# GloryyrolG/MHEntropy

Hardware: AMD Instinct MI355X
Metric: hypotheses/sec (BxK) fwd+loss, 256x256 (higher is better)
Workload: dtype bf16; 1 GPU; c2: MHEnt.get_loss forward+loss, resnet50 encoder (train-mode BN), 12-coupling RealNVP h=512, MANO joints, B=256/GPU, K=64, 256x256; images_per_gpu=256, hypotheses_per_image=64, global_batch=256, launch=hip-graph replay, base_noise=drawn on the device inside the step (Philox4x32-10, mhe_randn_f32), timing=one window of 452 steps, bracketed by barrier + synchronize, ranks=1, rccl_ranks=0

## Files before the change

mhentropy_amd/csrc/conv.hip:

```cpp
#include "conv_shared.h"
#include <cstdlib>

namespace mhe { namespace conv {

template <typename T, int BM, int BN, int WM, int WN, bool FAST, int MODE, bool DG = false>
__global__ __launch_bounds__(64 * WM * WN, WM * WN == 4 ? 2 : 1) void conv_kernel(const Params p) {
    constexpr int NTH = 64 * WM * WN;
    constexpr int CE = El<T>::CE, BKE = 8 * CE;
    constexpr int RSTEP = NTH / 8;
    constexpr int NJ_A = BM / RSTEP, NJ_B = BN / RSTEP;
    constexpr int MTW = BM / WM / 16, NTW = BN / WN / 16;
    __shared__ uint4 lds[2][(BM + BN) * 8];
    constexpr bool AFFM = MODE == 1 || MODE == 2;
    __shared__ __attribute__((aligned(16))) float aff[2][AFFM ? MAXC : 4];

    const int tid = threadIdx.x, wave = tid >> 6, lane = tid & 63;
    const int q = lane >> 4, l15 = lane & 15;
    const int wr = wave / WN, wc = wave % WN;
    int mtile, ntile;
    tile_of_block(mtile, ntile);
    const int m0 = mtile * BM, n0 = ntile * BN;
    const int s = tid & 7, rbase = tid >> 3;
    const T *xg = reinterpret_cast<const T *>(p.x);
    const T *wg = reinterpret_cast<const T *>(p.w);
// ... 657 lines not shown
extern "C" int mhe_conv1x1_cat_bias_nhwc(const mhe_conv_desc *d, const void *x, const void *xcat, int cin2, const void *w, void *y, const void *residual,
                                         const float *bias, void *stream) {
    MHE_REQUIRE(d && xcat && d->dtype == MHE_BF16 && d->KH == 1 && d->KW == 1 && d->stride == 1 && d->pad == 0 && cin2 > 0 && cin2 % 64 == 0 && d->Cin % 64 == 0,
                "mhe_conv1x1_cat_bias_nhwc: a bf16 1x1 stride-1 launch on two operand tensors with Cin and cin2 multiples of 64");
    MHE_REQUIRE(d->tile == 0 || d->tile == 1 || d->tile == 2, "mhe_conv1x1_cat_bias_nhwc: 128-row register-staged tiles only (tile 0, 1 or 2)");
    ConvRequest r;
    r.x = x; r.w = w; r.y = y; r.out_shift = bias; r.residual = residual; r.xcat = xcat; r.cin2 = cin2;
    return conv_entry(d, r, stream);
}

extern "C" int mhe_conv1x1_residual_in_masked_nhwc(const mhe_conv_desc *d, const void *x, const void *x2, const void *w, void *y,
                                                   const float *in_scale, const float *in_shift, const float *x2_scale,
                                                   const float *x2_shift, void *a_out, const void *residual, const void *mask,
                                                   const void *bn_y0, const float *bn_mean_invstd0, mhe_stat_t *bn_stats0, void *stream) {
    MHE_REQUIRE(d && x2 && in_scale && in_shift && mask, "mhe_conv1x1_residual_in_masked_nhwc: x2, in_scale, in_shift and mask are required");
    MHE_REQUIRE(d->KH == 1 && d->KW == 1 && d->stride == 1 && d->pad == 0, "mhe_conv1x1_residual_in_masked_nhwc: 1x1 stride-1 only");
    MHE_REQUIRE((x2_scale == nullptr) == (x2_shift == nullptr), "mhe_conv1x1_residual_in_masked_nhwc: x2_scale/x2_shift must come together");
    ConvRequest r;
    r.x = x; r.w = w; r.y = y; r.in_scale = in_scale; r.in_shift = in_shift; r.x2 = x2; r.x2_scale = x2_scale; r.x2_shift = x2_shift; r.a_out = a_out;
    if (int rc = bn_rev(r.bn, "mhe_conv1x1_residual_in_masked_nhwc", 1, {{bn_y0}, {bn_mean_invstd0}, {bn_stats0}})) return rc;
    MHE_REQUIRE(d->tile == 0 || d->tile == 1 || d->tile == 2 || d->tile == 11,
                "mhe_conv1x1_residual_in_masked_nhwc: 128-row tiles only (tile 0, 1, 2, or 11 = the transfer-wave kernel)");
    r.residual = residual; r.mask = mask;
    return conv_entry(d, r, stream);
}

extern "C" int mhe_conv2d_masked_nhwc(const mhe_conv_desc *d, const void *x, const void *w, void *y, const void *residual,
                                      const void *mask, const void *bn_y0, const float *bn_mean_invstd0, mhe_stat_t *bn_stats0,
                                      const void *bn_y1, const float *bn_mean_invstd1, mhe_stat_t *bn_stats1, void *stream) {
    MHE_REQUIRE(mask, "mhe_conv2d_masked_nhwc: mask is required");
    ConvRequest r;
    if (int rc = bn_rev(r.bn, "mhe_conv2d_masked_nhwc", 2, {{bn_y0, bn_y1}, {bn_mean_invstd0, bn_mean_invstd1}, {bn_stats0, bn_stats1}})) return rc;
    r.x = x; r.w = w; r.y = y; r.residual = residual; r.mask = mask;
    return conv_entry(d, r, stream);
}

extern "C" int mhe_conv2d_masked_bits_nhwc(const mhe_conv_desc *d, const void *x, const void *w, void *y, const void *residual,
                                           const void *mask, const void *mask_bits, const void *bn_y0, const float *bn_mean_invstd0, mhe_stat_t *bn_stats0,
                                           const void *bn_y1, const float *bn_mean_invstd1, mhe_stat_t *bn_stats1, void *stream) {
    MHE_REQUIRE(mask, "mhe_conv2d_masked_bits_nhwc: mask is required (kernels without the bit path read it)");
    ConvRequest r;
    if (int rc = bn_rev(r.bn, "mhe_conv2d_masked_bits_nhwc", 2, {{bn_y0, bn_y1}, {bn_mean_invstd0, bn_mean_invstd1}, {bn_stats0, bn_stats1}})) return rc;
    MHE_REQUIRE(!mask_bits || (d && d->Cout % 8 == 0), "mhe_conv2d_masked_bits_nhwc: Cout must be a multiple of 8");
    r.x = x; r.w = w; r.y = y; r.residual = residual; r.mask = mask; r.mask_bits = mask_bits;
    return conv_entry(d, r, stream);
}

extern "C" int mhe_conv2d_masked_bias_nhwc(const mhe_conv_desc *d, const void *x, const void *xcat, int cin2, const void *w, void *y,
                                           const void *residual, const void *mask, const float *bias, const void *bn_y0,
                                           const float *bn_mean_invstd0, mhe_stat_t *bn_stats0, void *stream) {
    MHE_REQUIRE(mask && bias, "mhe_conv2d_masked_bias_nhwc: mask and bias are required");
    MHE_REQUIRE(!xcat || (d && d->dtype == MHE_BF16 && d->KH == 1 && d->KW == 1 && d->stride == 1 && d->pad == 0 && cin2 > 0 && cin2 % 64 == 0 && d->Cin % 64 == 0),
                "mhe_conv2d_masked_bias_nhwc: a concatenated operand needs a bf16 1x1 stride-1 launch with Cin and cin2 multiples of 64");
    ConvRequest r;
    if (int rc = bn_rev(r.bn, "mhe_conv2d_masked_bias_nhwc", 1, {{bn_y0}, {bn_mean_invstd0}, {bn_stats0}})) return rc;
    MHE_REQUIRE(d && (d->tile == 0 || d->tile == 1 || d->tile == 2), "mhe_conv2d_masked_bias_nhwc: 128-row register-staged tiles only (tile 0, 1 or 2)");
    r.x = x; r.w = w; r.y = y; r.out_shift = bias; r.residual = residual; r.mask = mask; r.xcat = xcat; r.cin2 = xcat ? cin2 : 0;
    return conv_entry(d, r, stream);
}

extern "C" int mhe_conv3x3s2_dgrad_nhwc(int B, int Ho, int Wo, int Cout, int Cin, int dtype, const void *gy, const void *const *w4,
                                        void *dx, const void *residual, const void *mask, const void *bn_y0,
                                        const float *bn_mean_invstd0, mhe_stat_t *bn_stats0, const void *bn_y1,
                                        const float *bn_mean_invstd1, mhe_stat_t *bn_stats1, int tile, void *stream) {
    MHE_REQUIRE(gy && w4 && dx && w4[0] && w4[1] && w4[2] && w4[3], "mhe_conv3x3s2_dgrad_nhwc: null pointer");
    MHE_REQUIRE((!bn_y0 || (bn_mean_invstd0 && bn_stats0 && mask)) && (!bn_y1 || (bn_y0 && bn_mean_invstd1 && bn_stats1)),
                "mhe_conv3x3s2_dgrad_nhwc: each bn_y needs its mean_invstd and stats (and the gate)");
    ConvRequest r;
    r.x = gy; r.y = dx; r.residual = residual; r.mask = mask;
    if (mask) r.bn = {{bn_y0, bn_y1}, {bn_mean_invstd0, bn_mean_invstd1}, {bn_stats0, bn_stats1}};
    for (int py = 0; py < 2; ++py)
        for (int px = 0; px < 2; ++px) {
            mhe_conv_desc d = {B, Ho, Wo, Cout, Cin, 1 + py, 1 + px, 1, 0, dtype, 0, 0, tile};
            const int sc[2] = {py, px};
            r.w = w4[2 * py + px]; r.scatter = sc;
            if (int rc = conv_entry(&d, r, stream)) return rc;
        }
    return MHE_OK;
}

extern "C" int mhe_conv1x1_stats_nhwc(const mhe_conv_desc *d, const void *x, const void *w, const float *in_scale, const float *in_shift,
                                      mhe_stat_t *stats, void *stream) {
    MHE_REQUIRE(d && x && w && stats, "mhe_conv1x1_stats_nhwc: null pointer");
    MHE_REQUIRE(d->dtype == MHE_BF16 && d->KH == 1 && d->KW == 1 && d->stride == 1 && d->pad == 0 && (d->Cin == 64 || d->Cin == 128 || d->Cin == 256) && d->Cout % 256 == 0,
                "mhe_conv1x1_stats_nhwc: bf16 1x1 stride-1 with 64 / 128 / 256 input channels and a multiple of 256 output channels");
    MHE_REQUIRE((in_scale == nullptr) == (in_shift == nullptr), "mhe_conv1x1_stats_nhwc: in_scale/in_shift must come together");
    conv::Params p{};
    p.x = x; p.w = w; p.y = nullptr; p.in_scale = in_scale; p.in_shift = in_shift; p.stats = stats;
    const long long M = conv::fill_geometry(p, *d);
    MHE_REQUIRE(M > 0 && M < (1ll << 31), "mhe_conv1x1_stats_nhwc: bad pixel count");
    p.relu_in = d->relu_in; p.force = 8; p.stats_only = 1;
    if (d->Cin == 256) {
        p.force = 11;
        MHE_REQUIRE(conv::wide_supports(p), "mhe_conv1x1_stats_nhwc: geometry not taken by the resident-slab kernel (M=%lld Cout=%d)", M, d->Cout);
        return conv::launch_wide(p, (hipStream_t)stream);
    }
    MHE_REQUIRE(conv::stream_supports(p), "mhe_conv1x1_stats_nhwc: geometry not taken by the streaming kernel");
    return conv::launch_stream(p, (hipStream_t)stream);
}

extern "C" int mhe_bottleneck_tail_supported(const mhe_conv_desc *d, int Cb) {
    if (!d || d->dtype != MHE_BF16) return 0;
    static const float dummy = 0.f;
    conv::Params p{};
    p.x = p.x2 = p.w = p.w3 = p.y = p.a_out = (void *)&dummy; p.in_scale = p.in_shift = p.mid_scale = p.mid_shift = &dummy;
    const long long M = conv::fill_geometry(p, *d, true);
    if (M <= 0 || M >= (1ll << 31)) return 0;
    return conv::fuse_supports(p, Cb) ? 1 : 0;
}

static int bottleneck_tail(const char *entry, const mhe_conv_desc *d, int Cb, conv::Params &p, void *stream) {
    MHE_REQUIRE(d && p.x && p.in_scale && p.in_shift && p.w3 && p.mid_scale && p.mid_shift && p.x2 && p.w && p.a_out && p.y, "%s: null pointer", entry);
    MHE_REQUIRE(d->dtype == MHE_BF16, "%s: bf16 storage only", entry);
    MHE_REQUIRE((p.x2_scale == nullptr) == (p.x2_shift == nullptr), "%s: id_scale/id_shift must come together", entry);
    MHE_REQUIRE(!p.a_quarter || (d->B > 0 && d->H > 0 && d->W > 0), "%s: bad geometry", entry);
    p.relu_in = 1; p.force = -1;
    const long long M = conv::fill_geometry(p, *d, true);
    MHE_REQUIRE(M > 0 && (p.a_quarter ? M * d->Cin : M) < (1ll << 31), "%s: bad pixel count", entry);
    MHE_REQUIRE(conv::fuse_supports(p, Cb), "%s: needs Cin = 4 Cb, Cb 64 / 128, Cout 64 / 128, pixels %% 128 == 0 (Cin=%d Cb=%d Cout=%d M=%lld)",
                entry, d->Cin, Cb, d->Cout, M);
    return conv::launch_fuse(p, Cb, (hipStream_t)stream);
}

extern "C" int mhe_bottleneck_tail_nhwc(const mhe_conv_desc *d, int Cb, const void *y2, const float *bn2_scale, const float *bn2_shift,
                                        const void *w3, const float *bn3_scale, const float *bn3_shift, const void *identity,
                                        const float *id_scale, const float *id_shift, const void *w1, void *a_out, void *y1, mhe_stat_t *stats,
                                        void *stream) {
    return mhe_bottleneck_tail_bits_nhwc(d, Cb, y2, bn2_scale, bn2_shift, w3, bn3_scale, bn3_shift, identity, id_scale, id_shift, w1, a_out, nullptr, y1, stats, stream);
}

extern "C" int mhe_bottleneck_tail_bits_nhwc(const mhe_conv_desc *d, int Cb, const void *y2, const float *bn2_scale, const float *bn2_shift,
                                             const void *w3, const float *bn3_scale, const float *bn3_shift, const void *identity,
                                             const float *id_scale, const float *id_shift, const void *w1, void *a_out, void *a_bits, void *y1,
                                             mhe_stat_t *stats, void *stream) {
    conv::Params p{};
    p.x = y2; p.in_scale = bn2_scale; p.in_shift = bn2_shift; p.w3 = w3; p.mid_scale = bn3_scale; p.mid_shift = bn3_shift;
    p.x2 = identity; p.x2_scale = id_scale; p.x2_shift = id_shift; p.w = w1; p.a_out = a_out; p.y = y1; p.stats = stats;
    p.a_bits = (unsigned char *)a_bits;
    return bottleneck_tail("mhe_bottleneck_tail_nhwc", d, Cb, p, stream);
}

extern "C" int mhe_bottleneck_tail_quarter_nhwc(const mhe_conv_desc *d, int Cb, const void *y2, const float *bn2_scale, const float *bn2_shift,
                                                const void *w3, const float *bn3_scale, const float *bn3_shift, const void *identity,
                                                const float *id_scale, const float *id_shift, const void *w1, void *a_quarter, void *y1,
                                                mhe_stat_t *stats, void *stream) {
    conv::Params p{};
    p.x = y2; p.in_scale = bn2_scale; p.in_shift = bn2_shift; p.w3 = w3; p.mid_scale = bn3_scale; p.mid_shift = bn3_shift;
    p.x2 = identity; p.x2_scale = id_scale; p.x2_shift = id_shift; p.w = w1; p.a_out = a_quarter; p.y = y1; p.stats = stats;
    p.a_quarter = 1;
    return bottleneck_tail("mhe_bottleneck_tail_quarter_nhwc", d, Cb, p, stream);
}

extern "C" int mhe_conv_stat_shards(void) { return conv::NSH; }
extern "C" size_t mhe_stat_words(int C) { return C > 0 ? (size_t)2 * conv::NSH * 2 * (size_t)C : 0; }

extern "C" int mhe_conv_tile_mode(const mhe_conv_desc *d, int mode) {
    if (!d || mode < 0 || mode > 3) return -1;
    static const float dummy = 0.f;
    conv::Params p{};
    conv::fill_geometry(p, *d);
    p.force = d->tile - 1;
    if (mode == 1 || mode == 2) p.in_scale = &dummy;
    if (mode == 2) p.x2 = &dummy;
    if (mode == 3) p.residual = &dummy;
    return conv::choose_tile(p, d->Cin % (8 * conv::elem_chunk(d->dtype)) == 0, d->dtype == MHE_BF16);
}

// ... 244 lines not shown
```

mhentropy_amd/csrc/conv_wide.hip:

```cpp
#include "conv_shared.h"

namespace mhe { namespace conv {

namespace {
constexpr int WBM = 128, WBK = 64, WSLAB = 64 * 1024 / 16;
constexpr int WNSET = 8;
typedef unsigned int u32x4 __attribute__((ext_vector_type(4)));
}

template <int NS, int NK, bool BNLOAD>
__global__ __launch_bounds__(512) void conv_wide_kernel(const Params p, int nslab, int tiles_per_wg) {
    using T = u16;
    constexpr int CPR = NS / 8;
    constexpr int TPI = WNSET / NK;
    __shared__ uint4 Wl[WSLAB];
    __shared__ uint4 Al[3][WBM * 8];
    __shared__ uint4 Ol[WBM * CPR];
    __shared__ float aff[BNLOAD ? 2 * 512 : 2];
    const int tid = threadIdx.x, wave = __builtin_amdgcn_readfirstlane(tid >> 6), lane = tid & 63, q = lane >> 4, l15 = lane & 15;
    const bool mult = wave < 4;
    const int t2 = tid & 255, s = t2 & 7, rbase = t2 >> 3;
    constexpr int K = NK * WBK;
    const int xcd = blockIdx.x & 7, a = blockIdx.x >> 3, slab = a % nslab, group = a / nslab, ngroup = 32 / nslab;
    const int n0 = slab * NS;
    const int niter = tiles_per_wg / TPI;
    auto tile_m0 = [&](int j) __attribute__((always_inline)) { return (8 * (group + ngroup * j) + xcd) * WBM; };
    const T *xg = reinterpret_cast<const T *>(p.x), *wg = reinterpret_cast<const T *>(p.w);
    for (int i = tid; i < NS * NK * 8; i += 512) {
        const int c = i & 7, n = (i >> 3) % NS, kt = i / (8 * NS);
        Wl[kt * NS * 8 + swz(n, c)] = *reinterpret_cast<const uint4 *>(wg + (size_t)(n0 + n) * p.Kpad + kt * WBK + c * 8);
    }
    if constexpr (BNLOAD) {
        for (int i = tid; i < K; i += 512) { aff[i] = p.in_scale[i]; aff[512 + i] = p.in_shift[i]; }
    }
    __syncthreads();
    const bool st_on = p.stats != nullptr;
    constexpr int RSTEP = 256 / CPR, NR = WBM / RSTEP;
    float ss1[8], ss2[8];
#pragma unroll
    for (int e = 0; e < 8; ++e) ss1[e] = ss2[e] = 0.f;
    if (mult) {
        constexpr int MT = NS == 128 ? 4 : 2;
        const int px0 = NS == 128 ? (wave >> 1) * 64 : wave * 32, ch0 = NS == 128 ? (wave & 1) * 64 : 0;
        v4f acc[4][MT];
        uint4 fa[2][2][MT], fb[2][2][4];
        auto read_frags = [&](int buf, const uint4 *At, int kt) __attribute__((always_inline)) {
            const uint4 *Wt = Wl + kt * NS * 8;
#pragma unroll
            for (int kk = 0; kk < 2; ++kk) {
#pragma unroll
                for (int n = 0; n < 4; ++n) fb[buf][kk][n] = Wt[swz(ch0 + n * 16 + l15, kk * 4 + q)];
#pragma unroll
                for (int m = 0; m < MT; ++m) fa[buf][kk][m] = At[swz(px0 + m * 16 + l15, kk * 4 + q)];
            }
        };
        __syncthreads();
        read_frags(0, Al[0], 0);
        int sn = 1;
        for (int it = 0; it < niter; ++it) {
#pragma unroll
            for (int i = 0; i < WNSET; ++i) {
                const int kt = i % NK;
                if (kt == 0) {
#pragma unroll
                    for (int n = 0; n < 4; ++n)
#pragma unroll
                        for (int m = 0; m < MT; ++m) acc[n][m] = v4f{0.f, 0.f, 0.f, 0.f};
                }
                __syncthreads();
                read_frags((i + 1) & 1, Al[sn], (i + 1) % NK);
                sn = sn == 2 ? 0 : sn + 1;
                __builtin_amdgcn_sched_barrier(0);
#pragma unroll
                for (int kk = 0; kk < 2; ++kk)
#pragma unroll
                    for (int m = 0; m < MT; ++m)
#pragma unroll
                        for (int n = 0; n < 4; ++n)
                            acc[n][m] = __builtin_amdgcn_mfma_f32_16x16x32_bf16(
                                __builtin_bit_cast(__attribute__((ext_vector_type(8))) __bf16, fb[i & 1][kk][n]),
                                __builtin_bit_cast(__attribute__((ext_vector_type(8))) __bf16, fa[i & 1][kk][m]), acc[n][m], 0, 0, 0);
                __builtin_amdgcn_sched_barrier(0);
                if (kt == NK - 1) {
                    unsigned char *ot = reinterpret_cast<unsigned char *>(Ol);
#pragma unroll
                    for (int n = 0; n < 4; ++n)
#pragma unroll
                        for (int m = 0; m < MT; ++m) {
                            const int row = px0 + m * 16 + l15, boff = (ch0 + n * 16 + 4 * q) * 2;
                            const int chunk = (boff >> 4) ^ (row & (CPR - 1));
                            const v4f v = acc[n][m];
                            uint2 o;
                            o.x = (unsigned)f32_to_bf16(v[0]) | ((unsigned)f32_to_bf16(v[1]) << 16);
                            o.y = (unsigned)f32_to_bf16(v[2]) | ((unsigned)f32_to_bf16(v[3]) << 16);
                            *reinterpret_cast<uint2 *>(ot + ((size_t)row * CPR + chunk) * 16 + (boff & 15)) = o;
                        }
                }
            }
        }
        __syncthreads();
    } else {
        struct Set { uint4 a[4]; };
        Set st[WNSET];
        const __amdgpu_buffer_rsrc_t yrs = __builtin_amdgcn_make_buffer_rsrc(p.y ? p.y : const_cast<void *>(p.x), 0, p.y ? (int)((size_t)p.M * p.Cout * 2) : 0, 0x00020000);
        auto load_tick = [&](int j, int kt, Set &S) __attribute__((always_inline)) {
            const size_t m0 = (size_t)tile_m0(j < tiles_per_wg ? j : tiles_per_wg - 1);
#pragma unroll
            for (int i = 0; i < 4; ++i) S.a[i] = *reinterpret_cast<const uint4 *>(xg + (m0 + rbase + 32 * i) * K + kt * WBK + s * 8);
        };
        auto store_tick = [&](int stage, int kt, const Set &S) __attribute__((always_inline)) {
            uint4 *At = Al[stage];
            float sc[8], sh[8];
            if constexpr (BNLOAD) {
#pragma unroll
                for (int h = 0; h < 2; ++h) {
                    const float4 a0 = *reinterpret_cast<const float4 *>(aff + kt * WBK + s * 8 + 4 * h);
                    const float4 a1 = *reinterpret_cast<const float4 *>(aff + 512 + kt * WBK + s * 8 + 4 * h);
                    sc[4 * h] = a0.x; sc[4 * h + 1] = a0.y; sc[4 * h + 2] = a0.z; sc[4 * h + 3] = a0.w;
                    sh[4 * h] = a1.x; sh[4 * h + 1] = a1.y; sh[4 * h + 2] = a1.z; sh[4 * h + 3] = a1.w;
                }
            }
            const float lo = p.relu_in ? 0.f : -3.0e38f;
#pragma unroll
            for (int i = 0; i < 4; ++i) {
                uint4 v = S.a[i];
                if constexpr (BNLOAD) {
                    float f[8];
                    Chunk<T>::unpack(v, f);
#pragma unroll
                    for (int e = 0; e < 8; ++e) f[e] = fmaxf(fmaf(f[e], sc[e], sh[e]), lo);
                    v = Chunk<T>::pack(f);
                }
                At[swz(rbase + 32 * i, s)] = v;
            }
        };
        const int cc = t2 % CPR, r0 = t2 / CPR;
        auto epilogue = [&](int j, bool valid) __attribute__((always_inline)) {
            const unsigned char *ot = reinterpret_cast<const unsigned char *>(Ol);
            const unsigned m0 = (unsigned)tile_m0(valid ? j : 0);
            uint4 raw[NR];
#pragma unroll
            for (int i = 0; i < NR; ++i) {
                const int row = r0 + RSTEP * i;
                raw[i] = *reinterpret_cast<const uint4 *>(ot + ((size_t)row * CPR + (cc ^ (row & (CPR - 1)))) * 16);
            }
#pragma unroll
            for (int i = 0; i < NR; ++i) {
                const int row = r0 + RSTEP * i;
                if (st_on && valid) {
                    float f[8];
                    Chunk<T>::unpack(raw[i], f);
#pragma unroll
                    for (int e = 0; e < 8; ++e) { ss1[e] += f[e]; ss2[e] = fmaf(f[e], f[e], ss2[e]); }
                }
                const unsigned off = ((m0 + row) * (unsigned)p.Cout + n0 + cc * 8) * 2u;
                const u32x4 v = {raw[i].x, raw[i].y, raw[i].z, raw[i].w};
                __builtin_amdgcn_raw_buffer_store_b128(v, yrs, valid ? (int)off : (int)0x80000000u, 0, 0);
            }
        };
#pragma unroll
        for (int u = 0; u < WNSET; ++u) load_tick(u / NK, u % NK, st[u]);
        store_tick(0, 0, st[0]);
        load_tick(WNSET / NK, 0, st[0]);
        store_tick(1, 1 % NK, st[1]);
        load_tick((WNSET + 1) / NK, 1 % NK, st[1]);
        __syncthreads();
        int sw = 2;
        for (int it = 0; it < niter; ++it) {
#pragma unroll
            for (int i = 0; i < WNSET; ++i) {
                __syncthreads();
                store_tick(sw, (i + 2) % NK, st[(i + 2) % WNSET]);
                sw = sw == 2 ? 0 : sw + 1;
                if (i % NK == 0) epilogue(it * TPI + i / NK - 1, it * TPI + i / NK - 1 >= 0);
                load_tick(it * TPI + (i + 2 + WNSET) / NK, (i + 2) % NK, st[(i + 2) % WNSET]);
            }
        }
        __syncthreads();
        epilogue(tiles_per_wg - 1, true);
    }
    if (st_on) {
        __syncthreads();
        float *red = reinterpret_cast<float *>(Al);
        if (!mult) {
#pragma unroll
            for (int e = 0; e < 8; ++e) { red[t2 * 16 + e] = ss1[e]; red[t2 * 16 + 8 + e] = ss2[e]; }
        }
        __syncthreads();
        if (!mult && t2 < NS) {
            const int ch = t2 >> 3, e = t2 & 7;
            float a1 = 0.f, b1 = 0.f;
            for (int k = 0; k < RSTEP; ++k) { a1 += red[(ch + CPR * k) * 16 + e]; b1 += red[(ch + CPR * k) * 16 + 8 + e]; }
            fx::add(p.stats, (int)(blockIdx.x % NSH), 0, p.Cout, n0 + t2, a1);
            fx::add(p.stats, (int)(blockIdx.x % NSH), 1, p.Cout, n0 + t2, b1);
        }
    }
}

static int wide_ns(const Params &p) { return p.Cin == 256 ? 128 : 64; }

bool wide_supports(const Params &p) {
    if (!(p.KH == 1 && p.KW == 1 && p.stride == 1 && p.pad == 0 && (p.Cin == 256 || p.Cin == 512) && p.Kpad == p.Cin && !p.x2 && !p.mask &&
          !p.residual && !p.out_scale && !p.out_shift && !p.relu_out && !p.y32 && !p.os2 && !p.res_s2 && !p.a_out && p.M % WBM == 0))
        return false;
    const int ns = wide_ns(p);
    if (p.Cout % ns) return false;
    const int nslab = p.Cout / ns, gm = p.M / WBM;
    if (nslab < 4 || nslab > 32 || (32 % nslab) || gm % (256 / nslab)) return false;
    const int tiles = gm / (256 / nslab);
    if ((size_t)p.M * p.Cout * 2 >= (1ull << 31)) return false;
    return tiles >= 4 && tiles % (p.Cin == 256 ? 2 : 1) == 0;
}

int launch_wide(const Params &p, hipStream_t s) {
    const int ns = wide_ns(p), nslab = p.Cout / ns, tiles = (p.M / WBM) / (256 / nslab);
    const dim3 grid(256), block(512);
    if (ns == 128) {
        if (p.in_scale) hipLaunchKernelGGL((conv_wide_kernel<128, 4, true>), grid, block, 0, s, p, nslab, tiles);
        else hipLaunchKernelGGL((conv_wide_kernel<128, 4, false>), grid, block, 0, s, p, nslab, tiles);
    } else {
        if (p.in_scale) hipLaunchKernelGGL((conv_wide_kernel<64, 8, true>), grid, block, 0, s, p, nslab, tiles);
        else hipLaunchKernelGGL((conv_wide_kernel<64, 8, false>), grid, block, 0, s, p, nslab, tiles);
    }
    return check_launch("conv_wide_kernel");
}

}}
```

mhentropy_amd/ops.py:

```python
import ctypes as C
import os

import numpy as np
import torch

from . import _lib
from ._lib import ConvDesc, check

F32, BF16 = 0, 1
FLOW_FORWARD, FLOW_INVERSE = 0, 1

TIMING = False
TIMING_DG = False
KERNEL_TIMES = []


def _stream():
    return C.c_void_p(torch.cuda.current_stream().cuda_stream)


def _ptr(t):
    return C.c_void_p(0 if t is None else t.data_ptr())


# ... 24 lines not shown
    def __init__(self, what):
        self.what = what if TIMING else None

    def __enter__(self):
        if self.what is not None:
            self.rec = self.what()
            self.ev0, self.ev1 = torch.cuda.Event(enable_timing=True), torch.cuda.Event(enable_timing=True)
            self.ev0.record()
        return self

    def __exit__(self, exc_type, *exc):
        if self.what is not None and exc_type is None:
            self.ev1.record()
            name, flops, nbytes = self.rec
            KERNEL_TIMES.append((name, flops, self.ev0, self.ev1, nbytes))
        return False


def _bn_consumers(bn, n, dt, shape, Cn, prefix, only_one=None):
    bn = list(bn or [])
    if only_one and len(bn) > 1:
        raise ValueError(only_one)
    flat = []
    for by, bmi, bst in (bn + [(None, None, None)] * n)[:n]:
        if by is not None:
            _chk(by, dt, prefix + ".bn_y", shape); _chk(bmi, torch.float32, prefix + ".bn_mean_invstd", (2, Cn))
            _chk_stats(bst, prefix + ".bn_stats", Cn)
        flat += [by, bmi, bst]
    return flat


def _grow_only_workspace():
    live, retired = {}, []

    def get(device, need):
        ws = live.get(device)
        if ws is None or ws.numel() < need:
            if ws is not None:
                retired.append(ws)
            ws = live[device] = torch.empty(need, device=device, dtype=torch.float32)
        return ws
    return get


def stat_shards():
    return _lib.lib().mhe_conv_stat_shards()


STAT_DTYPE = torch.int64


def stat_shape(C):
    return (2, stat_shards(), 2, C)


def stat_unit(C, device):
    return torch.zeros(stat_shape(C), device=device, dtype=STAT_DTYPE)


def stat_totals(st):
    t = st.sum(1)
    return t[0].double() * 2.0 ** -16 + t[1].double() * 2.0 ** -56


def stat_from_float(t):
    d = t.double() * 2.0 ** 16
    hi = torch.round(d)
    lo = torch.round((d - hi) * 2.0 ** 40)
    return torch.stack([hi.to(torch.int64), lo.to(torch.int64)]).contiguous()


def _chk_stats(t, name, C):
    _chk(t, STAT_DTYPE, name, stat_shape(C))


_TILES = {0: "128, 64, 2, 2", 1: "128, 128, 2, 2", 2: "256, 256, 2, 4", 3: "256, 128, 4, 2", 4: "256, 64, 4, 2"}


def _conv_kernel_name(d, dt, mode):
    bke = 32 if dt == torch.float32 else 64
    tile = _lib.lib().mhe_conv_tile_mode(C.byref(d), mode)
    mode = 0 if mode == 3 else mode
    if tile == 11:
        return "mhe::conv::conv_wide_kernel<%s, %s>" % ("128, 4" if d.Cin == 256 else "64, 8", "true" if mode == 1 else "false")
    if tile == 10:
        return "mhe::conv::conv_tail_kernel<false>"
    if tile == 9:
        return "mhe::conv::conv3x3_c64_roles3_kernel<true>" if mode == 1 else "mhe::conv::conv3x3_c64_stream_kernel<false, false>"
    if tile == 8:
        return "mhe::conv::conv1x1_stream_kernel<%d, %d, %s, false>" % (d.Cin // 64, 64 if (d.Cin == 64 and d.Cout == 64) else 256 if d.Cin <= 128 else 128, "true" if mode == 1 else "false")
    if tile == 13:
        return "mhe::conv::conv_p8_kernel<false, %s, 0, 1>" % ("false" if d.KH == 1 and d.KW == 1 and d.pad == 0 else "true")
    if tile == 7:
        return "mhe::conv::conv_p8_kernel<false, %s, 0, 2>" % ("false" if d.KH == 1 and d.KW == 1 and d.pad == 0 else "true")
    return "mhe::conv::conv_kernel<%s, %s, %s, %d, false>" % ("float" if dt == torch.float32 else "unsigned short",
                                                             _TILES[tile],
                                                             "true" if d.Cin % bke == 0 else "false", mode)


def dtype_code(dt):
    return F32 if dt == torch.float32 else BF16


def conv_tile_choice(B, H, W, Cin, Cout, k, stride, pad, dt, mode=0):
    d = ConvDesc(B, H, W, Cin, Cout, k, k, stride, pad, dtype_code(dt), int(mode == 1), 0, 0, 0)
    return _lib.lib().mhe_conv_tile_mode(C.byref(d), mode)


def linear(x, w, bias=None, relu=False, out=None, want_bf16=False):
    M, K = x.shape
    N = w.shape[0]
    _chk(x, torch.float32, "linear.x"); _chk(w, torch.float32, "linear.w", (N, K))
    if bias is not None:
        _chk(bias, torch.float32, "linear.bias", (N,))
    y = out if out is not None else torch.empty(M, N, device=x.device, dtype=torch.float32)
    _chk(y, torch.float32, "linear.out", (M, N))
    if want_bf16:
        if M <= 256 and K % 64 == 0 and N % 4 == 0:
            yb = torch.empty(M, N, device=x.device, dtype=torch.bfloat16)
            launch("mhe_linear_f32_bf16copy", x, w, bias, y, yb, M, N, K, int(relu))
            return y, yb
        launch("mhe_linear_f32", x, w, bias, y, M, N, K, int(relu))
        return y, None
    launch("mhe_linear_f32", x, w, bias, y, M, N, K, int(relu))
    return y


_RNG_STATE = {}


def rng_state(device, seed=None):
    device = torch.device(device)
    if device.type == "cuda" and device.index is None:
        device = torch.device("cuda", torch.cuda.current_device())
    st = _RNG_STATE.get(device)
    if st is None:
        s = torch.initial_seed() if seed is None else int(seed)
        st = _RNG_STATE[device] = torch.tensor([s & 0x7FFFFFFFFFFFFFFF, 0, 0], dtype=torch.int64, device=device)
    elif seed is not None:
        st.copy_(torch.tensor([int(seed) & 0x7FFFFFFFFFFFFFFF, 0, 0], dtype=torch.int64))
    return st


def rng_get_state(device):
    return rng_state(device).cpu().clone()


def rng_set_state(device, words):
    st = rng_state(device)
    st.copy_(torch.as_tensor(words, dtype=torch.int64).reshape(3))
    return st


def randn(rows, cols, device, scale=1.0, state=None):
    out = torch.empty(rows, cols, device=device, dtype=torch.float32)
    st = state if state is not None else rng_state(out.device)
    launch("mhe_randn_f32", out, out.numel(), st, float(scale))
    return out


def dropout_(x, p, bits=None, state=None):
    if x.dtype not in (torch.float32, torch.bfloat16) or not x.is_cuda or not x.is_contiguous() or x.numel() % 8:
        raise _lib.MheError("dropout_: contiguous f32 / bf16 device tensor with a multiple of 8 elements expected")
    draw = bits is None
    if draw:
        bits = torch.empty(x.numel() // 8, device=x.device, dtype=torch.uint8)
# ... 461 lines not shown
        if B < 1 or R % B:
            raise ValueError(f"render_mesh: R={R} rows are not a multiple of the B={B} target images")
    if R < 1 or V < 1 or F < 1:
        raise ValueError(f"render_mesh: R={R} V={V} F={F} (each >= 1)")
    lo, hi = _faces_index_range(faces)
    if lo < 0 or hi >= V:
        raise ValueError(f"render_mesh: faces index {lo}..{hi} outside the V={V} vertices")
    shapes = {"mask": (R, S, S), "depth": (R, S, S), "iou_sums": (R, 2)}
    o = {k: (torch.empty(shapes[k], device=verts.device, dtype=torch.float32) if k in want else None) for k in RENDER_OUTPUTS}
    launch("mhe_render_mesh_f32", verts, faces, scale, trans, zscale, target, o["mask"], o["depth"], o["iou_sums"], R, B, V, F, S, int(bool(anti_aliasing)),
           float(far))
    return {k: v for k, v in o.items() if v is not None}


def conv2d_nhwc(x, w, KH, KW, stride, pad, in_scale=None, in_shift=None, relu_in=False, out_scale=None,
                out_shift=None, residual=None, relu_out=False, stats=None, out=None, mask=None, bn=None, tile=0, res_half=False, xcat=None,
                mask_bits=None):
    B, H, W, Cin = x.shape
    Cout = w.shape[0]
    dt = x.dtype
    _chk(x, dt, "conv.x"); _chk(w, dt, "conv.w")
    Ho, Wo = (H + 2 * pad - KH) // stride + 1, (W + 2 * pad - KW) // stride + 1
    y = out if out is not None else torch.empty(B, Ho, Wo, Cout, device=x.device, dtype=dt)
    _chk(y, dt, "conv.y", (B, Ho, Wo, Cout))
    for t, n, c in ((in_scale, "in_scale", Cin), (in_shift, "in_shift", Cin), (out_scale, "out_scale", Cout),
                    (out_shift, "out_shift", Cout)):
        if t is not None:
            _chk(t, torch.float32, "conv." + n, (c,))
    if residual is not None:
        _chk(residual, dt, "conv.residual", (B, (Ho + 1) // 2, (Wo + 1) // 2, Cout) if res_half else (B, Ho, Wo, Cout))
    if stats is not None:
        _chk_stats(stats, "conv.stats", Cout)
    d = ConvDesc(B, H, W, Cin, Cout, KH, KW, stride, pad, dtype_code(dt), int(relu_in), int(relu_out), int(tile), int(res_half))
    if mask is not None:
        if in_scale is not None or out_scale is not None or stats is not None or relu_in or relu_out:
            raise ValueError("conv2d_nhwc: mask= is the plain data-gradient form (no affine / statistics / relu; out_shift = a per-channel constant)")
        _chk(mask, dt, "conv.mask", (B, Ho, Wo, Cout))
        if out_shift is not None:
            ext = _bn_consumers(bn, 1, dt, y.shape, Cout, "conv", only_one="conv2d_nhwc: out_shift= with mask= takes one bn consumer")
            cin2 = 0
            if xcat is not None:
                cin2 = xcat.shape[-1]
                _chk(xcat, dt, "conv.xcat", (B, H, W, cin2))
                if tuple(w.shape) != (Cout, Cin + cin2):
                    raise ValueError(f"conv2d_nhwc: xcat= needs w [{Cout}, {Cin + cin2}], got {tuple(w.shape)}")
            with _dg_timed(d, x, y, w, residual, mask, None, ext[:1], "cat" if xcat is not None else "bias", xcat):
                launch("mhe_conv2d_masked_bias_nhwc", C.byref(d), x, xcat, int(cin2), w, y, residual, mask, out_shift, *ext)
            return y
        if xcat is not None:
            raise ValueError("conv2d_nhwc: xcat= comes with mask= and out_shift=")
        ext = _bn_consumers(bn, 2, dt, y.shape, Cout, "conv")
        if mask_bits is not None:
            _chk(mask_bits, torch.uint8, "conv.mask_bits", (B, Ho, Wo, Cout // 8))
            with _dg_timed(d, x, y, w, residual, mask, mask_bits, [b[0] for b in (bn or [])], "bits"):
                launch("mhe_conv2d_masked_bits_nhwc", C.byref(d), x, w, y, residual, mask, mask_bits, *ext)
            return y
        with _dg_timed(d, x, y, w, residual, mask, None, [b[0] for b in (bn or [])], ""):
            launch("mhe_conv2d_masked_nhwc", C.byref(d), x, w, y, residual, mask, *ext)
        return y
    if bn:
        raise ValueError("conv2d_nhwc: bn= needs mask= (data-gradient form)")
    if xcat is not None:
        if in_scale is not None or out_scale is not None or stats is not None or relu_in or relu_out:
            raise ValueError("conv2d_nhwc: xcat= without mask= takes out_shift and residual only")
        cin2 = xcat.shape[-1]
        _chk(xcat, dt, "conv.xcat", (B, H, W, cin2))
        if tuple(w.shape) != (Cout, Cin + cin2):
            raise ValueError(f"conv2d_nhwc: xcat= needs w [{Cout}, {Cin + cin2}], got {tuple(w.shape)}")
        launch("mhe_conv1x1_cat_bias_nhwc", C.byref(d), x, xcat, int(cin2), w, y, residual, out_shift)
        return y
    with _Timed(lambda: (_conv_kernel_name(d, dt, 1 if in_scale is not None else 3 if residual is not None else 0), 2.0 * B * Ho * Wo * Cout * KH * KW * Cin,
                         x.element_size() * (x.numel() + y.numel() + w.numel() + (residual.numel() if residual is not None else 0)))):
        launch("mhe_conv2d_nhwc", C.byref(d), x, w, y, in_scale, in_shift, out_scale, out_shift, residual, stats)
    return y


def conv1x1_stats(x, w, in_scale, in_shift, stats):
    B, H, W, Cin = x.shape
    Cout = w.shape[0]
    _chk(x, torch.bfloat16, "conv_stats.x"); _chk(w, torch.bfloat16, "conv_stats.w", (Cout, Cin))
    _chk(in_scale, torch.float32, "conv_stats.in_scale", (Cin,)); _chk(in_shift, torch.float32, "conv_stats.in_shift", (Cin,))
    _chk_stats(stats, "conv_stats.stats", Cout)
    d = ConvDesc(B, H, W, Cin, Cout, 1, 1, 1, 0, BF16, 1, 0, 0, 0)
    name = "mhe::conv::conv_wide_kernel<128, 4, true>" if Cin == 256 else "mhe::conv::conv1x1_stream_kernel<%d, 256, true, false>" % (Cin // 64)
    with _Timed(lambda: (name, 2.0 * B * H * W * Cout * Cin, 2 * (x.numel() + w.numel()))):
        launch("mhe_conv1x1_stats_nhwc", C.byref(d), x, w, in_scale, in_shift, stats)
    return stats


def gram_buffers(Cb, device):
    L = _lib.lib()
    return (torch.zeros(L.mhe_gram_stats_words(Cb), device=device, dtype=STAT_DTYPE),
            torch.empty(L.mhe_gram_stats_workspace_bytes(Cb) // 8, device=device, dtype=torch.float64))


def conv1x1_gram_bn(x, in_scale, in_shift, w, bn_weight, bn_bias, running_mean, running_var, bufs, momentum=0.1, eps=1e-5, num_batches_tracked=None,
                    want_mean_invstd=False, a_out=None):
    B, H, W, Cb = x.shape
    Cn = w.shape[0]
    _chk(x, torch.bfloat16, "gram.x"); _chk(w, torch.bfloat16, "gram.w", (Cn, Cb))
    _chk(in_scale, torch.float32, "gram.in_scale", (Cb,)); _chk(in_shift, torch.float32, "gram.in_shift", (Cb,))
    gram, ws = bufs
    L = _lib.lib()
    _chk(gram, STAT_DTYPE, "gram.accumulators", (L.mhe_gram_stats_words(Cb),))
    if a_out is not None:
        _chk(a_out, torch.bfloat16, "gram.a_out", (B, H, W, Cb))
    with _Timed(lambda: ("mhe::conv::gram_kernel<%d>" % Cb, 2.0 * B * H * W * Cb * Cb, 2 * x.numel())):
        launch("mhe_conv1x1_gram_store_nhwc", x, in_scale, in_shift, 1, gram, a_out, B * H * W, Cb)
    scale = torch.empty(Cn, device=x.device, dtype=torch.float32)
    shift = torch.empty_like(scale)
    mi = torch.empty(2, Cn, device=x.device, dtype=torch.float32) if want_mean_invstd else None
    launch("mhe_gram_bn_finalize", gram, ws, w, bn_weight, bn_bias, running_mean, running_var, scale, shift, mi, Cn, Cb, float(B * H * W), float(momentum),
           float(eps), num_batches_tracked)
    return (scale, shift, mi) if want_mean_invstd else (scale, shift)


def gram_workspace(Cb, device):
    return torch.empty(_lib.lib().mhe_gram_stats_workspace_bytes(Cb) // 8, device=device, dtype=torch.float64)


def conv3_bn_fold(D, w, gram_totals, rev_stats, gamma, mean_invstd, count, dgamma, dbeta, dW, w_dg, S, c0, coef_ws):
    Cn, Cb = w.shape
    if S is None:
        _chk(w_dg, torch.bfloat16, "fold.w_cat", (Cb, Cn + Cb))
        s_ptr, ld_s = C.c_void_p(w_dg.data_ptr() + 2 * Cn), Cn + Cb
    else:
        _chk(S, torch.bfloat16, "fold.S", (Cb, Cb))
        s_ptr, ld_s = S, Cb
    _chk(D, torch.float32, "fold.D", (Cn, Cb)); _chk(w, torch.bfloat16, "fold.w", (Cn, Cb)); _chk(gram_totals, torch.float64, "fold.gram")
    _chk_stats(rev_stats, "fold.rev_stats", Cn); _chk(gamma, torch.float32, "fold.gamma", (Cn,))
    _chk(mean_invstd, torch.float32, "fold.mean_invstd", (2, Cn)); _chk(dgamma, torch.float32, "fold.dgamma", (Cn,)); _chk(dbeta, torch.float32, "fold.dbeta", (Cn,))
    _chk(dW, torch.float32, "fold.dW"); _chk(w_dg, torch.bfloat16, "fold.w_dg")
    _chk(c0, torch.float32, "fold.c0", (Cb,)); _chk(coef_ws, torch.float32, "fold.coef_ws")
    if gram_totals.numel() < Cb * Cb + Cb or dW.numel() < Cn * Cb or w_dg.shape[0] != Cb or w_dg.shape[1] < Cn or coef_ws.numel() < 2 * Cn:
        raise ValueError("conv3_bn_fold: operand sizes")
    launch("mhe_conv3_bn_fold", D, w, gram_totals, rev_stats, gamma, mean_invstd, float(count), dgamma, dbeta, dW, w_dg, int(w_dg.shape[1]), s_ptr, int(ld_s), c0,
           coef_ws, Cn, Cb)


def conv3x3_halo_supported(B, H, W, Cin, Cout):
    return bool(_lib.lib().mhe_conv3x3_halo_supported(int(B), int(H), int(W), int(Cin), int(Cout)))


def conv3x3_halo_pack(w):
    _chk(w, torch.bfloat16, "halo_pack.w")
    Cout, K = w.shape
    if K % 9 or (K // 9) % 64 or Cout % 128:
        raise ValueError(f"conv3x3_halo_pack: weight rows [{Cout}][{K}] are not 9 x (a multiple of 64) wide / a multiple of 128 many")
    out = torch.empty_like(w)
    launch("mhe_conv3x3_halo_pack_bf16", w, out, int(Cout), int(K // 9))
    return out


def conv3x3_halo(x, w_halo, in_scale=None, in_shift=None, relu_in=False, a_out=None, stats=None, residual=None, mask=None, bn=None):
    B, H, W, Cin = x.shape
    Cout = w_halo.shape[0]
    _chk(x, torch.bfloat16, "halo.x"); _chk(w_halo, torch.bfloat16, "halo.w", (Cout, 9 * Cin))
    y = torch.empty(B, H, W, Cout, device=x.device, dtype=torch.bfloat16)
    for t, name, shape in ((in_scale, "in_scale", (Cin,)), (in_shift, "in_shift", (Cin,))):
        if t is not None:
            _chk(t, torch.float32, "halo." + name, shape)
    if stats is not None:
        _chk_stats(stats, "halo.stats", Cout)
    for t, name, shape in ((a_out, "a_out", tuple(x.shape)), (residual, "residual", tuple(y.shape)), (mask, "mask", tuple(y.shape))):
        if t is not None:
            _chk(t, torch.bfloat16, "halo." + name, shape)
    ext = _bn_consumers(None if bn is None else [bn], 1, torch.bfloat16, y.shape, Cout, "halo")
# ... 914 lines not shown
```

Baseline: 2.597 million hypotheses/s.

## Split wide conv into loader, MMA and storer wave roles for BN-load path

Adds a three-role variant of the resident-slab 1x1 conv kernel (768 threads) for the Cin=256 BN-load case. A separate group of storer waves runs the epilogue and stats, so loader waves only stage inputs. The MMA waves drop to single-buffered fragments and interleave half-K LDS reads with MFMAs, which cuts register pressure. It also allows tile counts that do not divide evenly, clamping the last tile and masking duplicate rows, so the kernel covers more geometries. The cost is more threads per workgroup and extra barriers for the storer waves.

```diff
diff --git a/mhentropy_amd/csrc/conv.hip b/mhentropy_amd/csrc/conv.hip
--- a/mhentropy_amd/csrc/conv.hip
+++ b/mhentropy_amd/csrc/conv.hip
@@ -763,7 +763,7 @@
 extern "C" int mhe_conv1x1_stats_nhwc(const mhe_conv_desc *d, const void *x, const void *w, const float *in_scale, const float *in_shift,
                                       mhe_stat_t *stats, void *stream) {
     MHE_REQUIRE(d && x && w && stats, "mhe_conv1x1_stats_nhwc: null pointer");
-    MHE_REQUIRE(d->dtype == MHE_BF16 && d->KH == 1 && d->KW == 1 && d->stride == 1 && d->pad == 0 && (d->Cin == 64 || d->Cin == 128 || d->Cin == 256) && d->Cout % 256 == 0,
+    MHE_REQUIRE(d->dtype == MHE_BF16 && d->KH == 1 && d->KW == 1 && d->stride == 1 && d->pad == 0 && (d->Cin == 64 || d->Cin == 128 || d->Cin == 256) && d->Cout % (d->Cin == 256 ? 128 : 256) == 0,
                 "mhe_conv1x1_stats_nhwc: bf16 1x1 stride-1 with 64 / 128 / 256 input channels and a multiple of 256 output channels");
     MHE_REQUIRE((in_scale == nullptr) == (in_shift == nullptr), "mhe_conv1x1_stats_nhwc: in_scale/in_shift must come together");
     conv::Params p{};
diff --git a/mhentropy_amd/csrc/conv_wide.hip b/mhentropy_amd/csrc/conv_wide.hip
--- a/mhentropy_amd/csrc/conv_wide.hip
+++ b/mhentropy_amd/csrc/conv_wide.hip
@@ -8,9 +8,11 @@
 typedef unsigned int u32x4 __attribute__((ext_vector_type(4)));
 }
 
-template <int NS, int NK, bool BNLOAD>
-__global__ __launch_bounds__(512) void conv_wide_kernel(const Params p, int nslab, int tiles_per_wg) {
+template <int NS, int NK, bool BNLOAD, int ROLES>
+__device__ __forceinline__ void conv_wide_body(const Params &p, int nslab, int tiles_per_wg) {
+    static_assert(ROLES == 2 || (ROLES == 3 && BNLOAD), "the plain form keeps its two roles");
     using T = u16;
+    constexpr int NTH = 256 * ROLES;
     constexpr int CPR = NS / 8;
     constexpr int TPI = WNSET / NK;
     __shared__ uint4 Wl[WSLAB];
@@ -19,19 +21,22 @@
     __shared__ float aff[BNLOAD ? 2 * 512 : 2];
     const int tid = threadIdx.x, wave = __builtin_amdgcn_readfirstlane(tid >> 6), lane = tid & 63, q = lane >> 4, l15 = lane & 15;
     const bool mult = wave < 4;
+    const bool loader = !mult && (ROLES == 2 || wave < 8), storer = !mult && (ROLES == 2 || wave >= 8);
     const int t2 = tid & 255, s = t2 & 7, rbase = t2 >> 3;
     constexpr int K = NK * WBK;
     const int xcd = blockIdx.x & 7, a = blockIdx.x >> 3, slab = a % nslab, group = a / nslab, ngroup = 32 / nslab;
     const int n0 = slab * NS;
-    const int niter = tiles_per_wg / TPI;
-    auto tile_m0 = [&](int j) __attribute__((always_inline)) { return (8 * (group + ngroup * j) + xcd) * WBM; };
+    const int niter = (tiles_per_wg + TPI - 1) / TPI;
+    const int gm = (p.M + WBM - 1) / WBM;
+    auto tile_ok = [&](int j) __attribute__((always_inline)) { return j >= 0 && j < tiles_per_wg && 8 * (group + ngroup * j) + xcd < gm; };
+    auto tile_m0 = [&](int j) __attribute__((always_inline)) { return tile_ok(j) ? min((8 * (group + ngroup * j) + xcd) * WBM, p.M - WBM) : 0; };
     const T *xg = reinterpret_cast<const T *>(p.x), *wg = reinterpret_cast<const T *>(p.w);
-    for (int i = tid; i < NS * NK * 8; i += 512) {
+    for (int i = tid; i < NS * NK * 8; i += NTH) {
         const int c = i & 7, n = (i >> 3) % NS, kt = i / (8 * NS);
         Wl[kt * NS * 8 + swz(n, c)] = *reinterpret_cast<const uint4 *>(wg + (size_t)(n0 + n) * p.Kpad + kt * WBK + c * 8);
     }
     if constexpr (BNLOAD) {
-        for (int i = tid; i < K; i += 512) { aff[i] = p.in_scale[i]; aff[512 + i] = p.in_shift[i]; }
+        for (int i = tid; i < K; i += NTH) { aff[i] = p.in_scale[i]; aff[512 + i] = p.in_shift[i]; }
     }
     __syncthreads();
     const bool st_on = p.stats != nullptr;
@@ -43,20 +48,32 @@
         constexpr int MT = NS == 128 ? 4 : 2;
         const int px0 = NS == 128 ? (wave >> 1) * 64 : wave * 32, ch0 = NS == 128 ? (wave & 1) * 64 : 0;
         v4f acc[4][MT];
-        uint4 fa[2][2][MT], fb[2][2][4];
+        constexpr int NB = ROLES == 3 ? 1 : 2;
+        uint4 fa[NB][2][MT], fb[NB][2][4];
+        auto read_half = [&](int buf, int kk, const uint4 *At, int kt) __attribute__((always_inline)) {
+            const uint4 *Wt = Wl + kt * NS * 8;
+#pragma unroll
+            for (int n = 0; n < 4; ++n) fb[buf][kk][n] = Wt[swz(ch0 + n * 16 + l15, kk * 4 + q)];
+#pragma unroll
+            for (int m = 0; m < MT; ++m) fa[buf][kk][m] = At[swz(px0 + m * 16 + l15, kk * 4 + q)];
+        };
         auto read_frags = [&](int buf, const uint4 *At, int kt) __attribute__((always_inline)) {
-            const uint4 *Wt = Wl + kt * NS * 8;
-#pragma unroll
-            for (int kk = 0; kk < 2; ++kk) {
-#pragma unroll
-                for (int n = 0; n < 4; ++n) fb[buf][kk][n] = Wt[swz(ch0 + n * 16 + l15, kk * 4 + q)];
-#pragma unroll
-                for (int m = 0; m < MT; ++m) fa[buf][kk][m] = At[swz(px0 + m * 16 + l15, kk * 4 + q)];
-            }
-        };
-        __syncthreads();
-        read_frags(0, Al[0], 0);
-        int sn = 1;
+#pragma unroll
+            for (int kk = 0; kk < 2; ++kk) read_half(buf, kk, At, kt);
+        };
+        auto mfma_half = [&](int buf, int kk) __attribute__((always_inline)) {
+#pragma unroll
+            for (int m = 0; m < MT; ++m)
+#pragma unroll
+                for (int n = 0; n < 4; ++n)
+                    acc[n][m] = __builtin_amdgcn_mfma_f32_16x16x32_bf16(
+                        __builtin_bit_cast(__attribute__((ext_vector_type(8))) __bf16, fb[buf][kk][n]),
+                        __builtin_bit_cast(__attribute__((ext_vector_type(8))) __bf16, fa[buf][kk][m]), acc[n][m], 0, 0, 0);
+        };
+        __syncthreads();
+        if constexpr (ROLES == 3) read_half(0, 0, Al[0], 0);
+        else read_frags(0, Al[0], 0);
+        int sc = 0, sn = 1;
         for (int it = 0; it < niter; ++it) {
 #pragma unroll
             for (int i = 0; i < WNSET; ++i) {
@@ -68,18 +85,22 @@
                         for (int m = 0; m < MT; ++m) acc[n][m] = v4f{0.f, 0.f, 0.f, 0.f};
                 }
                 __syncthreads();
-                read_frags((i + 1) & 1, Al[sn], (i + 1) % NK);
+                if constexpr (ROLES == 3) {
+                    read_half(0, 1, Al[sc], kt);
+                    __builtin_amdgcn_sched_barrier(0);
+                    mfma_half(0, 0);
+                    __builtin_amdgcn_sched_barrier(0);
+                    read_half(0, 0, Al[sn], (i + 1) % NK);
+                    __builtin_amdgcn_sched_barrier(0);
+                    mfma_half(0, 1);
+                } else {
+                    read_frags((i + 1) & 1, Al[sn], (i + 1) % NK);
+                    __builtin_amdgcn_sched_barrier(0);
+#pragma unroll
+                    for (int kk = 0; kk < 2; ++kk) mfma_half(i & 1, kk);
+                }
+                sc = sn;
                 sn = sn == 2 ? 0 : sn + 1;
-                __builtin_amdgcn_sched_barrier(0);
-#pragma unroll
-                for (int kk = 0; kk < 2; ++kk)
-#pragma unroll
-                    for (int m = 0; m < MT; ++m)
-#pragma unroll
-                        for (int n = 0; n < 4; ++n)
-                            acc[n][m] = __builtin_amdgcn_mfma_f32_16x16x32_bf16(
-                                __builtin_bit_cast(__attribute__((ext_vector_type(8))) __bf16, fb[i & 1][kk][n]),
-                                __builtin_bit_cast(__attribute__((ext_vector_type(8))) __bf16, fa[i & 1][kk][m]), acc[n][m], 0, 0, 0);
                 __builtin_amdgcn_sched_barrier(0);
                 if (kt == NK - 1) {
                     unsigned char *ot = reinterpret_cast<unsigned char *>(Ol);
@@ -104,7 +125,7 @@
         Set st[WNSET];
         const __amdgpu_buffer_rsrc_t yrs = __builtin_amdgcn_make_buffer_rsrc(p.y ? p.y : const_cast<void *>(p.x), 0, p.y ? (int)((size_t)p.M * p.Cout * 2) : 0, 0x00020000);
         auto load_tick = [&](int j, int kt, Set &S) __attribute__((always_inline)) {
-            const size_t m0 = (size_t)tile_m0(j < tiles_per_wg ? j : tiles_per_wg - 1);
+            const size_t m0 = (size_t)tile_m0(j);
 #pragma unroll
             for (int i = 0; i < 4; ++i) S.a[i] = *reinterpret_cast<const uint4 *>(xg + (m0 + rbase + 32 * i) * K + kt * WBK + s * 8);
         };
@@ -135,9 +156,11 @@
             }
         };
         const int cc = t2 % CPR, r0 = t2 / CPR;
-        auto epilogue = [&](int j, bool valid) __attribute__((always_inline)) {
+        auto epilogue = [&](int j) __attribute__((always_inline)) {
             const unsigned char *ot = reinterpret_cast<const unsigned char *>(Ol);
-            const unsigned m0 = (unsigned)tile_m0(valid ? j : 0);
+            const bool valid = tile_ok(j);
+            const unsigned m0 = (unsigned)tile_m0(j);
+            const int rlo = valid ? (8 * (group + ngroup * j) + xcd) * WBM - (int)m0 : WBM;
             uint4 raw[NR];
 #pragma unroll
             for (int i = 0; i < NR; ++i) {
@@ -147,7 +170,8 @@
 #pragma unroll
             for (int i = 0; i < NR; ++i) {
                 const int row = r0 + RSTEP * i;
-                if (st_on && valid) {
+                const bool own = row >= rlo;
+                if (st_on && own) {
                     float f[8];
                     Chunk<T>::unpack(raw[i], f);
 #pragma unroll
@@ -155,39 +179,54 @@
                 }
                 const unsigned off = ((m0 + row) * (unsigned)p.Cout + n0 + cc * 8) * 2u;
                 const u32x4 v = {raw[i].x, raw[i].y, raw[i].z, raw[i].w};
-                __builtin_amdgcn_raw_buffer_store_b128(v, yrs, valid ? (int)off : (int)0x80000000u, 0, 0);
-            }
-        };
-#pragma unroll
-        for (int u = 0; u < WNSET; ++u) load_tick(u / NK, u % NK, st[u]);
-        store_tick(0, 0, st[0]);
-        load_tick(WNSET / NK, 0, st[0]);
-        store_tick(1, 1 % NK, st[1]);
-        load_tick((WNSET + 1) / NK, 1 % NK, st[1]);
-        __syncthreads();
-        int sw = 2;
-        for (int it = 0; it < niter; ++it) {
-#pragma unroll
-            for (int i = 0; i < WNSET; ++i) {
-                __syncthreads();
-                store_tick(sw, (i + 2) % NK, st[(i + 2) % WNSET]);
-                sw = sw == 2 ? 0 : sw + 1;
-                if (i % NK == 0) epilogue(it * TPI + i / NK - 1, it * TPI + i / NK - 1 >= 0);
-                load_tick(it * TPI + (i + 2 + WNSET) / NK, (i + 2) % NK, st[(i + 2) % WNSET]);
-            }
-        }
-        __syncthreads();
-        epilogue(tiles_per_wg - 1, true);
+                __builtin_amdgcn_raw_buffer_store_b128(v, yrs, own ? (int)off : (int)0x80000000u, 0, 0);
+            }
+        };
+        if (loader) {
+#pragma unroll
+            for (int u = 0; u < WNSET; ++u) load_tick(u / NK, u % NK, st[u]);
+            store_tick(0, 0, st[0]);
+            load_tick(WNSET / NK, 0, st[0]);
+            store_tick(1, 1 % NK, st[1]);
+            load_tick((WNSET + 1) / NK, 1 % NK, st[1]);
+            __syncthreads();
+            int sw = 2;
+            for (int it = 0; it < niter; ++it) {
+#pragma unroll
+                for (int i = 0; i < WNSET; ++i) {
+                    __syncthreads();
+                    store_tick(sw, (i + 2) % NK, st[(i + 2) % WNSET]);
+                    sw = sw == 2 ? 0 : sw + 1;
+                    if constexpr (ROLES == 2) {
+                        if (i % NK == 0) epilogue(it * TPI + i / NK - 1);
+                    }
+                    load_tick(it * TPI + (i + 2 + WNSET) / NK, (i + 2) % NK, st[(i + 2) % WNSET]);
+                }
+            }
+            __syncthreads();
+            if constexpr (ROLES == 2) epilogue(niter * TPI - 1);
+        } else {
+            __syncthreads();
+            for (int it = 0; it < niter; ++it) {
+#pragma unroll
+                for (int i = 0; i < WNSET; ++i) {
+                    __syncthreads();
+                    if (i % NK == 0) epilogue(it * TPI + i / NK - 1);
+                }
+            }
+            __syncthreads();
+            epilogue(niter * TPI - 1);
+        }
     }
     if (st_on) {
         __syncthreads();
         float *red = reinterpret_cast<float *>(Al);
-        if (!mult) {
+        if (storer) {
 #pragma unroll
             for (int e = 0; e < 8; ++e) { red[t2 * 16 + e] = ss1[e]; red[t2 * 16 + 8 + e] = ss2[e]; }
         }
         __syncthreads();
-        if (!mult && t2 < NS) {
+        if (storer && t2 < NS) {
             const int ch = t2 >> 3, e = t2 & 7;
             float a1 = 0.f, b1 = 0.f;
             for (int k = 0; k < RSTEP; ++k) { a1 += red[(ch + CPR * k) * 16 + e]; b1 += red[(ch + CPR * k) * 16 + 8 + e]; }
@@ -197,26 +236,33 @@
     }
 }
 
+template <int NS, int NK, bool BNLOAD>
+__global__ __launch_bounds__(512) void conv_wide_kernel(const Params p, int nslab, int tiles_per_wg) { conv_wide_body<NS, NK, BNLOAD, 2>(p, nslab, tiles_per_wg); }
+template <int NS, int NK>
+__global__ __launch_bounds__(768) void conv_wide_roles3_kernel(const Params p, int nslab, int tiles_per_wg) { conv_wide_body<NS, NK, true, 3>(p, nslab, tiles_per_wg); }
+
 static int wide_ns(const Params &p) { return p.Cin == 256 ? 128 : 64; }
 
 bool wide_supports(const Params &p) {
     if (!(p.KH == 1 && p.KW == 1 && p.stride == 1 && p.pad == 0 && (p.Cin == 256 || p.Cin == 512) && p.Kpad == p.Cin && !p.x2 && !p.mask &&
-          !p.residual && !p.out_scale && !p.out_shift && !p.relu_out && !p.y32 && !p.os2 && !p.res_s2 && !p.a_out && p.M % WBM == 0))
+          !p.residual && !p.out_scale && !p.out_shift && !p.relu_out && !p.y32 && !p.os2 && !p.res_s2 && !p.a_out && p.M >= WBM))
         return false;
     const int ns = wide_ns(p);
     if (p.Cout % ns) return false;
-    const int nslab = p.Cout / ns, gm = p.M / WBM;
-    if (nslab < 4 || nslab > 32 || (32 % nslab) || gm % (256 / nslab)) return false;
+    const int nslab = p.Cout / ns, gm = (p.M + WBM - 1) / WBM;
+    if (nslab > 32 || (32 % nslab)) return false;
+    if ((size_t)p.M * p.Cout * 2 >= (1ull << 31)) return false;
+    if (p.force == 11) return true;
+    if (p.M % WBM || nslab < 4 || gm % (256 / nslab)) return false;
     const int tiles = gm / (256 / nslab);
-    if ((size_t)p.M * p.Cout * 2 >= (1ull << 31)) return false;
     return tiles >= 4 && tiles % (p.Cin == 256 ? 2 : 1) == 0;
 }
 
 int launch_wide(const Params &p, hipStream_t s) {
-    const int ns = wide_ns(p), nslab = p.Cout / ns, tiles = (p.M / WBM) / (256 / nslab);
+    const int ns = wide_ns(p), nslab = p.Cout / ns, per = 256 / nslab, tiles = ((p.M + WBM - 1) / WBM + per - 1) / per;
     const dim3 grid(256), block(512);
     if (ns == 128) {
-        if (p.in_scale) hipLaunchKernelGGL((conv_wide_kernel<128, 4, true>), grid, block, 0, s, p, nslab, tiles);
+        if (p.in_scale) hipLaunchKernelGGL((conv_wide_roles3_kernel<128, 4>), grid, dim3(768), 0, s, p, nslab, tiles);
         else hipLaunchKernelGGL((conv_wide_kernel<128, 4, false>), grid, block, 0, s, p, nslab, tiles);
     } else {
         if (p.in_scale) hipLaunchKernelGGL((conv_wide_kernel<64, 8, true>), grid, block, 0, s, p, nslab, tiles);
diff --git a/mhentropy_amd/ops.py b/mhentropy_amd/ops.py
--- a/mhentropy_amd/ops.py
+++ b/mhentropy_amd/ops.py
@@ -130,6 +130,8 @@
     tile = _lib.lib().mhe_conv_tile_mode(C.byref(d), mode)
     mode = 0 if mode == 3 else mode
     if tile == 11:
+        if d.Cin == 256 and mode == 1:
+            return "mhe::conv::conv_wide_roles3_kernel<128, 4>"
         return "mhe::conv::conv_wide_kernel<%s, %s>" % ("128, 4" if d.Cin == 256 else "64, 8", "true" if mode == 1 else "false")
     if tile == 10:
         return "mhe::conv::conv_tail_kernel<false>"
@@ -757,7 +759,7 @@
     _chk(in_scale, torch.float32, "conv_stats.in_scale", (Cin,)); _chk(in_shift, torch.float32, "conv_stats.in_shift", (Cin,))
     _chk_stats(stats, "conv_stats.stats", Cout)
     d = ConvDesc(B, H, W, Cin, Cout, 1, 1, 1, 0, BF16, 1, 0, 0, 0)
-    name = "mhe::conv::conv_wide_kernel<128, 4, true>" if Cin == 256 else "mhe::conv::conv1x1_stream_kernel<%d, 256, true, false>" % (Cin // 64)
+    name = "mhe::conv::conv_wide_roles3_kernel<128, 4>" if Cin == 256 else "mhe::conv::conv1x1_stream_kernel<%d, 256, true, false>" % (Cin // 64)
     with _Timed(lambda: (name, 2.0 * B * H * W * Cout * Cin, 2 * (x.numel() + w.numel()))):
         launch("mhe_conv1x1_stats_nhwc", C.byref(d), x, w, in_scale, in_shift, stats)
     return stats
```

Measured after the change: 2.596 million hypotheses/s. Within noise of the previous version (-0.1%).
